# DIAGNijmegen/bodyct-dram-emph-subtype

Measured on AMD Instinct MI355X. Metric: CT volumes/sec (train step, 1x128x256x256), higher is better.
Workload: dtype f32; 1 GPU; BASELINE configs[1]: resnet18segcls train step (fwd+loss+bwd+Adam), batch 2/GPU, 1x128x256x256, fp32, inputs resident in HBM; global_batch=2, parallelism=dp1, hip_graph=False, streams=2

## Files before the change

### bodyct-dram-emph-subtype_amd/csrc/bn.hip

```cpp
#include <stdlib.h>
#include <atomic>
#include "common.h"

namespace {

template <typename T>
__global__ void reduce_partials_kernel(const T* __restrict__ partial, double* __restrict__ out, int nparts,
                                       int RC, double tail, int has_tail) {
  __shared__ double sm[256];
  const int col = blockIdx.x * 64 + (threadIdx.x & 63);
  const int lane4 = threadIdx.x >> 6;
  const int S = gridDim.y, sidx = blockIdx.y;
  double s = 0.0;
  if (col < RC)
    for (int p = sidx + S * lane4; p < nparts; p += 4 * S) s += (double)partial[(long)p * RC + col];
  sm[threadIdx.x] = s;
  __syncthreads();
  if (lane4 == 0 && col < RC)
    out[(long)sidx * RC + col] = sm[threadIdx.x] + sm[threadIdx.x + 64] + sm[threadIdx.x + 128] + sm[threadIdx.x + 192];
  if (has_tail && blockIdx.x == 0 && blockIdx.y == 0 && threadIdx.x == 0) out[RC] = tail;
}

__global__ void bn_finalize_kernel(const double* __restrict__ sums, double count_host,
                                   const double* __restrict__ count_dev, const float* __restrict__ gamma,
                                   const float* __restrict__ beta, float* __restrict__ rmean,
                                   float* __restrict__ rvar, float momentum, float eps, int update,
                                   float* __restrict__ mean, float* __restrict__ invstd, float* __restrict__ scale,
                                   float* __restrict__ shift, int C) {
  const int c = blockIdx.x * blockDim.x + threadIdx.x;
  if (c >= C) return;
  double m, v;
  const double count = count_dev ? *count_dev : count_host;
  if (sums) {
    m = sums[c] / count;
    v = sums[C + c] / count - m * m;
    if (v < 0.0) v = 0.0;
    if (update) {
      const double unb = count > 1.0 ? v * (count / (count - 1.0)) : v;
      rmean[c] = (float)((1.0 - (double)momentum) * (double)rmean[c] + (double)momentum * m);
      rvar[c] = (float)((1.0 - (double)momentum) * (double)rvar[c] + (double)momentum * unb);
    }
  } else {
    m = (double)rmean[c];
    v = (double)rvar[c];
  }
  const double is = 1.0 / sqrt(v + (double)eps);
  const float sc = (float)((double)gamma[c] * is);
  mean[c] = (float)m;
  invstd[c] = (float)is;
  scale[c] = sc;
  shift[c] = (float)((double)beta[c] - m * (double)gamma[c] * is);
}

struct FoldFinalize {
  double count;
  const float* gamma; const float* beta; float* rmean; float* rvar;
  float momentum, eps; int update;
  float* mean; float* invstd; float* scale; float* shift;
};
constexpr int FOLD_XMAX = 512;

__global__ __launch_bounds__(1024) void fold_partials_kernel(const float* __restrict__ partial, double* scratch,
                                                             double* __restrict__ sums, float* __restrict__ sums_f32,
                                                             float* __restrict__ f32_row1, const int nparts, const int RC,
                                                             const double tail,
                                                             const int has_tail, unsigned* __restrict__ ticket,
                                                             const FoldFinalize ff) {
  __shared__ double sm[1024];
  __shared__ double tot[64];
  __shared__ unsigned s_ticket;
  const int t64 = threadIdx.x & 63, lane4 = threadIdx.x >> 6;
  const int C = RC >> 1;
  const int col = ff.gamma ? (t64 >> 5) * C + blockIdx.x * 32 + (t64 & 31) : blockIdx.x * 64 + t64;
  const bool live = ff.gamma ? (blockIdx.x * 32 + (t64 & 31) < C) : (col < RC);
  const int S = gridDim.y, sidx = blockIdx.y;
  double s = 0.0;
  if (live) {
    const int step = 16 * S;
    int p = sidx + S * lane4;
    for (; p + 7 * step < nparts; p += 8 * step) {
      float v[8];
#pragma unroll
      for (int j = 0; j < 8; ++j) v[j] = partial[(long)(p + j * step) * RC + col];
#pragma unroll
      for (int j = 0; j < 8; ++j) s += (double)v[j];
    }
    for (; p < nparts; p += step) s += (double)partial[(long)p * RC + col];
  }
  sm[threadIdx.x] = s;
  __syncthreads();
  double total = 0.0;
  if (lane4 == 0) {
#pragma unroll
    for (int j = 0; j < 16; ++j) total += sm[t64 + 64 * j];
  }
  if (S > 1) {
    if (lane4 == 0 && live) scratch[(long)sidx * RC + col] = total;
    __threadfence();
    __syncthreads();
    if (threadIdx.x == 0) s_ticket = atomicAdd(&ticket[blockIdx.x], 1u);
    __syncthreads();
    if (s_ticket != (unsigned)S - 1) return;
    __threadfence();
    if (lane4 == 0 && live) {
      total = 0.0;
      int k = 0;
      for (; k + 8 <= S; k += 8) {
        double v[8];
#pragma unroll
        for (int j = 0; j < 8; ++j)
          v[j] = __hip_atomic_load(scratch + (long)(k + j) * RC + col, __ATOMIC_RELAXED, __HIP_MEMORY_SCOPE_AGENT);
#pragma unroll
        for (int j = 0; j < 8; ++j) total += v[j];
      }
      for (; k < S; ++k)
        total += __hip_atomic_load(scratch + (long)k * RC + col, __ATOMIC_RELAXED, __HIP_MEMORY_SCOPE_AGENT);
    }
  }
  if (lane4 == 0 && live) {
    sums[col] = total;
    if (sums_f32) {
      if (f32_row1 && col >= C) f32_row1[col - C] = (float)total;
      else sums_f32[col] = (float)total;
    }
  }
  if (has_tail && blockIdx.x == 0 && threadIdx.x == 0) sums[RC] = tail;
  if (!ff.gamma) return;
  if (lane4 == 0) tot[t64] = total;
  __syncthreads();
  const int c = blockIdx.x * 32 + threadIdx.x;
  if (threadIdx.x < 32 && c < C) {
    const double m = tot[threadIdx.x] / ff.count;
    double v = tot[32 + threadIdx.x] / ff.count - m * m;
    if (v < 0.0) v = 0.0;
    if (ff.update) {
      const double unb = ff.count > 1.0 ? v * (ff.count / (ff.count - 1.0)) : v;
      ff.rmean[c] = (float)((1.0 - (double)ff.momentum) * (double)ff.rmean[c] + (double)ff.momentum * m);
      ff.rvar[c] = (float)((1.0 - (double)ff.momentum) * (double)ff.rvar[c] + (double)ff.momentum * unb);
    }
    const double is = 1.0 / sqrt(v + (double)ff.eps);
    ff.mean[c] = (float)m;
    ff.invstd[c] = (float)is;
    ff.scale[c] = (float)((double)ff.gamma[c] * is);
    ff.shift[c] = (float)((double)ff.beta[c] - m * (double)ff.gamma[c] * is);
  }
}

template <int RES, typename T>
__global__ void bn_apply_kernel(const T* __restrict__ y, const float* __restrict__ scale,
                                const float* __restrict__ shift, const T* __restrict__ res, int Cr, int rs,
                                T* __restrict__ z, int D, int H, int W, int C, long total4, int relu) {
  const int Q = C >> 2;
  for (long i = blockIdx.x * (long)blockDim.x + threadIdx.x; i < total4; i += (long)gridDim.x * blockDim.x) {
    const int q = (int)(i % Q);
    const float4 sc = *reinterpret_cast<const float4*>(scale + 4 * q);
    const float4 sh = *reinterpret_cast<const float4*>(shift + 4 * q);
    const float4 v = ld4<T>(y, 4 * i);
    float4 o;
    o.x = __builtin_fmaf(v.x, sc.x, sh.x); o.y = __builtin_fmaf(v.y, sc.y, sh.y);
    o.z = __builtin_fmaf(v.z, sc.z, sh.z); o.w = __builtin_fmaf(v.w, sc.w, sh.w);
    if (RES == 1) {
      const float4 rr = ld4<T>(res, 4 * i);
      o.x += rr.x; o.y += rr.y; o.z += rr.z; o.w += rr.w;
    }
    if (relu) { o.x = fmaxf(o.x, 0.f); o.y = fmaxf(o.y, 0.f); o.z = fmaxf(o.z, 0.f); o.w = fmaxf(o.w, 0.f); }
    st4<T>(z, 4 * i, o);
  }
}

template <int RES, typename T, int U>
__global__ __launch_bounds__(256) void bn_apply_fast_kernel(const T* __restrict__ y, const float* __restrict__ scale,
                                                            const float* __restrict__ shift, const T* __restrict__ res,
                                                            T* __restrict__ z, int Q, long total4, int relu) {
  const int q = threadIdx.x % Q;
  const float4 sc = *reinterpret_cast<const float4*>(scale + 4 * q);
  const float4 sh = *reinterpret_cast<const float4*>(shift + 4 * q);
  const long stride = (long)gridDim.x * 256;
  for (long i0 = blockIdx.x * 256L + threadIdx.x; i0 < total4; i0 += U * stride) {
    float4 v[U], rr[U];
#pragma unroll
    for (int u = 0; u < U; ++u) {
      const long i = i0 + u * stride;
      if (i < total4) {
        v[u] = ld4<T>(y, 4 * i);
        if (RES == 1) rr[u] = ld4<T>(res, 4 * i);
// ... 333 lines not shown
            gg.z = zv.z > 0.f ? gg.z : 0.f; gg.w = zv.w > 0.f ? gg.w : 0.f;
          }
          const float4 o = make_float4(sc.x * gg.x, sc.y * gg.y, sc.z * gg.z, sc.w * gg.w);
          st4<T>(dy, 4 * i, o);
          cs.x += o.x; cs.y += o.y; cs.z += o.z; cs.w += o.w;
        }
      }
    }
  }
  if (colpart) {
    __shared__ float4 sm[256];
    sm[threadIdx.x] = cs;
    __syncthreads();
    if ((int)threadIdx.x < Q) {
      float4 t = sm[threadIdx.x];
      for (int k = threadIdx.x + Q; k < 256; k += Q) {
        const float4 u = sm[k];
        t.x += u.x; t.y += u.y; t.z += u.z; t.w += u.w;
      }
      *reinterpret_cast<float4*>(colpart + (long)blockIdx.x * C + 4 * threadIdx.x) = t;
    }
  }
}

__global__ void add_kernel(const float4* __restrict__ a, const float4* __restrict__ b, float4* __restrict__ o,
                           long n4, const float* __restrict__ as, const float* __restrict__ bs,
                           float* __restrict__ os, long n) {
  for (long i = blockIdx.x * (long)blockDim.x + threadIdx.x; i < n4; i += (long)gridDim.x * blockDim.x) {
    const float4 u = a[i], v = b[i];
    o[i] = make_float4(u.x + v.x, u.y + v.y, u.z + v.z, u.w + v.w);
  }
  const long t0 = n4 * 4;
  for (long i = t0 + blockIdx.x * (long)blockDim.x + threadIdx.x; i < n; i += (long)gridDim.x * blockDim.x)
    os[i] = as[i] + bs[i];
}

inline int ew_grid(long total4) {
  long b = (total4 + 255) / 256;
  return (int)(b > 4096 ? 4096 : (b < 1 ? 1 : b));
}

inline int rows_per_block(long long rows) {
  long long rpb = (rows + 1023) / 1024;
  if (rpb < 64) rpb = 64;
  return (int)rpb;
}

}

extern "C" int dram_reduce_partials_stages(int nparts) {
  if (nparts <= 64) return 1;
  int s = (nparts + 31) / 32;
  return s > 64 ? 64 : s;
}

extern "C" int dram_reduce_partials(const float* partial, double* sums, double* scratch, int nparts, int R, int C,
                                    double tail, int has_tail, dram_stream_t stream) {
  if (!partial || !sums || nparts < 1 || R < 1 || C < 1) return DRAM_ERR_BAD_ARG;
  const int RC = R * C;
  const int S = dram_reduce_partials_stages(nparts);
  hipStream_t st = (hipStream_t)stream;
  DramProf prof(DRAM_FAM_BN, 0, 0.0, 4.0 * (double)nparts * RC + 8.0 * RC, st);
  if (S == 1) {
    hipLaunchKernelGGL((reduce_partials_kernel<float>), dim3((RC + 63) / 64, 1), dim3(256), 0, st, partial, sums,
                       nparts, RC, tail, has_tail);
  } else {
    if (!scratch) return DRAM_ERR_WORKSPACE;
    hipLaunchKernelGGL((reduce_partials_kernel<float>), dim3((RC + 63) / 64, S), dim3(256), 0, st, partial, scratch,
                       nparts, RC, 0.0, 0);
    DRAM_LAUNCH_CHECK();
    hipLaunchKernelGGL((reduce_partials_kernel<double>), dim3((RC + 63) / 64, 1), dim3(256), 0, st,
                       (const double*)scratch, sums, S, RC, tail, has_tail);
  }
  DRAM_LAUNCH_CHECK();
  return DRAM_OK;
}

extern "C" int dram_fold_partials_stages(int nparts) {
  if (nparts <= 1024) return 1;
  const int s = (nparts + 511) / 512;
  return s > 64 ? 64 : s;
}

static int fold_launch(const float* partial, double* sums, double* scratch, float* sums_f32, float* f32_row1, int nparts,
                       int RC, double tail, int has_tail, const FoldFinalize& ff, hipStream_t st) {
  const int S = dram_fold_partials_stages(nparts);
  const int gx = ff.gamma ? (RC / 2 + 31) / 32 : (RC + 63) / 64;
  if (S > 1 && gx > FOLD_XMAX) return DRAM_ERR_UNSUPPORTED;
  unsigned* ticket = nullptr;
  if (S > 1) {
    ticket = reinterpret_cast<unsigned*>(scratch + (long)S * RC);
    const hipError_t e = hipMemsetAsync(ticket, 0, sizeof(unsigned) * gx, st);
    if (e != hipSuccess) return (int)e;
  }
  DramProf prof(DRAM_FAM_BN, 0, 0.0, 4.0 * (double)nparts * RC + 8.0 * RC, st);
  hipLaunchKernelGGL(fold_partials_kernel, dim3(gx, S), dim3(1024), 0, st, partial, scratch, sums, sums_f32, f32_row1,
                     nparts, RC, tail, has_tail, ticket, ff);
  DRAM_LAUNCH_CHECK();
  return DRAM_OK;
}

extern "C" int dram_fold_partials(const float* partial, double* sums, double* scratch, float* sums_f32, float* f32_row1,
                                  int nparts, int R, int C, double tail, int has_tail, dram_stream_t stream) {
  if (!partial || !sums || !scratch || nparts < 1 || R < 1 || C < 1) return DRAM_ERR_BAD_ARG;
  if (f32_row1 && (R != 2 || !sums_f32)) return DRAM_ERR_BAD_ARG;
  FoldFinalize ff{};
  return fold_launch(partial, sums, scratch, sums_f32, f32_row1, nparts, R * C, tail, has_tail, ff, (hipStream_t)stream);
}

extern "C" int dram_bn_fold_finalize(const float* partial, double* sums, double* scratch, int nparts, int C, double count,
                                     const float* gamma, const float* beta, float* running_mean, float* running_var,
                                     float momentum, float eps, int update_running, float* mean, float* invstd,
                                     float* scale, float* shift, dram_stream_t stream) {
  if (!partial || !sums || !scratch || nparts < 1 || C < 1 || count <= 0.0) return DRAM_ERR_BAD_ARG;
  if (!gamma || !beta || !mean || !invstd || !scale || !shift) return DRAM_ERR_BAD_ARG;
  if (update_running && (!running_mean || !running_var)) return DRAM_ERR_BAD_ARG;
  FoldFinalize ff{count, gamma, beta, running_mean, running_var, momentum, eps, update_running, mean, invstd, scale, shift};
  return fold_launch(partial, sums, scratch, nullptr, nullptr, nparts, 2 * C, 0.0, 0, ff, (hipStream_t)stream);
}

extern "C" int dram_bn_finalize(const double* sums, double count, const double* count_dev, const float* gamma,
                                const float* beta,
                                float* running_mean, float* running_var, float momentum, float eps,
                                int update_running, float* mean, float* invstd, float* scale, float* shift, int C,
                                dram_stream_t stream) {
  if (!gamma || !beta || !mean || !invstd || !scale || !shift || C < 1) return DRAM_ERR_BAD_ARG;
  if (!sums && (!running_mean || !running_var)) return DRAM_ERR_BAD_ARG;
  if (sums && !count_dev && count <= 0.0) return DRAM_ERR_BAD_ARG;
  if (update_running && (!running_mean || !running_var)) return DRAM_ERR_BAD_ARG;
  DramProf prof(DRAM_FAM_BN, 1, 0.0, 4.0 * 10.0 * C, (hipStream_t)stream);
  hipLaunchKernelGGL(bn_finalize_kernel, dim3((C + 255) / 256), dim3(256), 0, (hipStream_t)stream, sums, count,
                     count_dev, gamma, beta, running_mean, running_var, momentum, eps, update_running, mean, invstd, scale,
                     shift, C);
  DRAM_LAUNCH_CHECK();
  return DRAM_OK;
}

template <typename T>
static int bn_apply_impl(const T* y, const float* scale, const float* shift, const T* residual, int Dr, int Hr, int Wr,
                         int Cr, int rs, T* z, int B, int D, int H, int W, int C, int relu, dram_stream_t stream) {
  if (!y || !scale || !shift || !z || B < 1 || D < 1 || H < 1 || W < 1 || C < 4 || (C & 3)) return DRAM_ERR_BAD_ARG;
  const long total4 = (long)B * D * H * W * (C >> 2);
  hipStream_t s = (hipStream_t)stream;
  const int grid = ew_blocks(total4, 256, 4096);
  const double res_frac = !residual ? 0.0 : ((double)Cr / C) / ((double)rs * rs * rs);
  DramProf prof(DRAM_FAM_BN, 2, 0.0, 4.0 * sizeof(T) * (double)total4 * (2.0 + res_frac), s);
  const int Q = C >> 2;
  const bool identity = residual && rs == 1 && Cr == C && Dr == D && Hr == H && Wr == W;
  static const int ew_u = tune_env("DRAM_EW_U") ? atoi(tune_env("DRAM_EW_U")) : 4;
  if ((!residual || identity) && 256 % Q == 0 && ew_u > 0 && ew_shape() > 0) {
    const int g1 = ew_blocks(total4, 1024, 0);
#define BN_SHOT_(RES_, NT_) hipLaunchKernelGGL((bn_apply_shot_kernel<RES_, T, NT_>), dim3(g1), dim3(256), 0, s, y, scale, \
                                               shift, residual, z, Q, total4, relu)
    const bool nt = ew_stream(sizeof(T) * 4 * total4);
    if (!residual) { if (nt) BN_SHOT_(0, true); else BN_SHOT_(0, false); }
    else           { if (nt) BN_SHOT_(1, true); else BN_SHOT_(1, false); }
#undef BN_SHOT_
  } else if ((!residual || identity) && 256 % Q == 0 && ew_u > 0) {
    const long per = (total4 + 255) / 256;
    const int g2 = (int)((per + ew_u - 1) / ew_u < 8192 ? ((per + ew_u - 1) / ew_u < 1 ? 1 : (per + ew_u - 1) / ew_u) : 8192);
#define BN_FAST_(RES_, U_) hipLaunchKernelGGL((bn_apply_fast_kernel<RES_, T, U_>), dim3(g2), dim3(256), 0, s, y, scale, shift, \
                                              residual, z, Q, total4, relu)
    if (!residual) { if (ew_u >= 4) BN_FAST_(0, 4); else if (ew_u >= 2) BN_FAST_(0, 2); else BN_FAST_(0, 1); }
    else           { if (ew_u >= 4) BN_FAST_(1, 4); else if (ew_u >= 2) BN_FAST_(1, 2); else BN_FAST_(1, 1); }
#undef BN_FAST_
  } else if (!residual) {
    hipLaunchKernelGGL((bn_apply_kernel<0, T>), dim3(grid), dim3(256), 0, s, y, scale, shift, (const T*)nullptr, 0,
                       1, z, D, H, W, C, total4, relu);
  } else if (identity) {
    hipLaunchKernelGGL((bn_apply_kernel<1, T>), dim3(grid), dim3(256), 0, s, y, scale, shift, residual,
                       Cr, 1, z, D, H, W, C, total4, relu);
  } else {
    if ((Cr & 3) || Cr < 4 || Cr > C || rs < 1) return DRAM_ERR_BAD_ARG;
    if ((D - 1) * rs >= Dr || (H - 1) * rs >= Hr || (W - 1) * rs >= Wr) return DRAM_ERR_BAD_ARG;
    hipLaunchKernelGGL((bn_apply_shortcut_a_kernel<T>), dim3(grid), dim3(256), 0, s, y, scale, shift,
                       residual, Dr, Hr, Wr, Cr, rs, z, D, H, W, C, total4, relu);
// ... 159 lines not shown
```

### bodyct-dram-emph-subtype_amd/csrc/common.h

```cpp
#pragma once
#include <hip/hip_runtime.h>
#include <stdint.h>
#include <stdlib.h>
#include "dram_hip.h"

typedef float f32x16 __attribute__((ext_vector_type(16)));
typedef float f32x4 __attribute__((ext_vector_type(4)));

#define DRAM_LAUNCH_CHECK()                         \
  do {                                              \
    hipError_t _e = hipGetLastError();              \
    if (_e != hipSuccess) return (int)_e;           \
  } while (0)

extern bool g_dram_prof_on;
void dram_prof_begin(int family, int variant, double mfma_flops, double hbm_bytes, double alg_flops, hipStream_t s);
void dram_prof_end(hipStream_t s);
struct DramProf {
  const bool on;
  hipStream_t s;
  DramProf(int family, int variant, double mfma_flops, double hbm_bytes, hipStream_t st, double alg_flops = -1.0)
      : on(g_dram_prof_on), s(st) {
    if (on) dram_prof_begin(family, variant, mfma_flops, hbm_bytes, alg_flops < 0.0 ? mfma_flops : alg_flops, st);
  }
// ... 43 lines not shown
template <> __device__ __forceinline__ fvec<4> ldv<float, 4>(const float* p, long off) {
  const float4 t = *reinterpret_cast<const float4*>(p + off);
  return fvec<4>{{t.x, t.y, t.z, t.w}};
}
template <> __device__ __forceinline__ fvec<4> ldv<bf16_t, 4>(const bf16_t* p, long off) {
  const uint2 u = *reinterpret_cast<const uint2*>(p + off);
  return fvec<4>{{__uint_as_float(u.x << 16), __uint_as_float(u.x & 0xffff0000u), __uint_as_float(u.y << 16),
                  __uint_as_float(u.y & 0xffff0000u)}};
}
template <> __device__ __forceinline__ fvec<8> ldv<bf16_t, 8>(const bf16_t* p, long off) {
  const uint4 u = *reinterpret_cast<const uint4*>(p + off);
  return fvec<8>{{__uint_as_float(u.x << 16), __uint_as_float(u.x & 0xffff0000u), __uint_as_float(u.y << 16),
                  __uint_as_float(u.y & 0xffff0000u), __uint_as_float(u.z << 16), __uint_as_float(u.z & 0xffff0000u),
                  __uint_as_float(u.w << 16), __uint_as_float(u.w & 0xffff0000u)}};
}
template <typename T, int VW> __device__ __forceinline__ void stv(T* p, long off, const fvec<VW>& a);
template <> __device__ __forceinline__ void stv<float, 4>(float* p, long off, const fvec<4>& a) {
  *reinterpret_cast<float4*>(p + off) = make_float4(a.v[0], a.v[1], a.v[2], a.v[3]);
}
template <> __device__ __forceinline__ void stv<bf16_t, 4>(bf16_t* p, long off, const fvec<4>& a) {
  *reinterpret_cast<uint2*>(p + off) = make_uint2(pack2_bf16(a.v[0], a.v[1]), pack2_bf16(a.v[2], a.v[3]));
}
template <> __device__ __forceinline__ void stv<bf16_t, 8>(bf16_t* p, long off, const fvec<8>& a) {
  *reinterpret_cast<uint4*>(p + off) = make_uint4(pack2_bf16(a.v[0], a.v[1]), pack2_bf16(a.v[2], a.v[3]),
                                                  pack2_bf16(a.v[4], a.v[5]), pack2_bf16(a.v[6], a.v[7]));
}

typedef float f32x4_nt __attribute__((ext_vector_type(4)));
typedef unsigned u32x2_nt __attribute__((ext_vector_type(2)));
template <typename T> __device__ __forceinline__ float4 ld4s(const T* p, long off);
template <> __device__ __forceinline__ float4 ld4s<float>(const float* p, long off) {
  const f32x4_nt t = __builtin_nontemporal_load(reinterpret_cast<const f32x4_nt*>(p + off));
  return make_float4(t.x, t.y, t.z, t.w);
}
template <> __device__ __forceinline__ float4 ld4s<bf16_t>(const bf16_t* p, long off) {
  const u32x2_nt u = __builtin_nontemporal_load(reinterpret_cast<const u32x2_nt*>(p + off));
  return make_float4(__uint_as_float(u.x << 16), __uint_as_float(u.x & 0xffff0000u), __uint_as_float(u.y << 16),
                     __uint_as_float(u.y & 0xffff0000u));
}
template <typename T> __device__ __forceinline__ void st4s(T* p, long off, float4 v);
template <> __device__ __forceinline__ void st4s<float>(float* p, long off, float4 v) {
  const f32x4_nt t = {v.x, v.y, v.z, v.w};
  __builtin_nontemporal_store(t, reinterpret_cast<f32x4_nt*>(p + off));
}
template <> __device__ __forceinline__ void st4s<bf16_t>(bf16_t* p, long off, float4 v) {
  const u32x2_nt t = {pack2_bf16(v.x, v.y), pack2_bf16(v.z, v.w)};
  __builtin_nontemporal_store(t, reinterpret_cast<u32x2_nt*>(p + off));
}

static inline const char* tune_env(const char* name) {
  static const bool on = [] { const char* t = getenv("DRAM_TUNING"); return t && t[0] == '1'; }();
  return on ? getenv(name) : nullptr;
}

static inline int ew_shape() {
  static const int v = tune_env("DRAM_EW_SHAPE") ? atoi(tune_env("DRAM_EW_SHAPE")) : 2;
  return v;
}
static inline bool ew_stream(long long tensor_bytes) { return ew_shape() >= 2 && tensor_bytes >= (256LL << 20); }
static inline int ew_blocks(long items, int per_block, int cap) {
  long b = (items + per_block - 1) / per_block;
  if (b < 1) b = 1;
  if (ew_shape() == 0 && b > cap) b = cap;
  return (int)(b > 0x7fffffffL ? 0x7fffffffL : b);
}

static inline int cdiv(long long a, long long b) { return (int)((a + b - 1) / b); }

__device__ __forceinline__ int xcd_remap(int bid, int nblk) {
  const int q = nblk >> 3, r = nblk & 7;
  const int xcd = bid & 7, idx = bid >> 3;
  return (xcd < r ? xcd * (q + 1) : r * (q + 1) + (xcd - r) * q) + idx;
}

__device__ __forceinline__ void lin_src(int dst, float scale, int in, int& i0, int& i1, float& w0, float& w1) {
  const float s = scale * (float)dst;
  i0 = (int)s;
  if (i0 > in - 1) i0 = in - 1;
  i1 = i0 + (i0 < in - 1 ? 1 : 0);
  w1 = s - (float)i0;
  w0 = 1.f - w1;
}

__device__ __forceinline__ float wave_sum(float v) {
#pragma unroll
  for (int o = 32; o > 0; o >>= 1) v += __shfl_xor(v, o, 64);
  return v;
}
```

### bodyct-dram-emph-subtype_amd/csrc/pool_up.hip

```cpp
#include <stdlib.h>
#include <string.h>
#include <initializer_list>
#include "common.h"

namespace {

inline int ew_grid(long total) { return ew_blocks(total, 256, 8192); }

template <typename T, int VW>
__global__ void maxpool_fwd_kernel(const T* __restrict__ x, T* __restrict__ y,
                                   uint8_t* __restrict__ amax, int D, int H, int W, int C, int Do, int Ho, int Wo,
                                   long total) {
  const int Q = C / VW;
  for (long i = blockIdx.x * (long)blockDim.x + threadIdx.x; i < total; i += (long)gridDim.x * blockDim.x) {
    const int q = (int)(i % Q);
    long v = i / Q;
    const int xo = (int)(v % Wo); v /= Wo;
    const int yo = (int)(v % Ho); v /= Ho;
    const int zo = (int)(v % Do);
    const long b = v / Do;
    fvec<VW> m;
    int am[VW];
#pragma unroll
    for (int k = 0; k < VW; ++k) { m.v[k] = -INFINITY; am[k] = 0; }
// ... 266 lines not shown
template <typename T, int VW>
__global__ __launch_bounds__(256) void upcat_fwd_tiled_kernel(const T* __restrict__ src, const T* __restrict__ skip,
                                                              T* __restrict__ cat, int Ds, int Hs, int Ws, int Cu,
                                                              int Dk, int Hk, int Wk, int Ck, int oz, int oy, int ox,
                                                              float sz, float sy, float sx, int tz_n, int ty_n,
                                                              int tx_n) {
  constexpr int LPV = 64 / VW;
  constexpr int SLOTS = 256 / LPV;
  __shared__ float4 tile[216 * 16];
  const int Do = 2 * Ds, Ho = 2 * Hs, Wo = 2 * Ws;
  const int Ct = Cu + Ck, Qk = Ck / VW;
  int r = blockIdx.x;
  const int txi = r % tx_n; r /= tx_n;
  const int tyi = r % ty_n; r /= ty_n;
  const int tzi = r % tz_n;
  const long b = r / tz_n;
  const int z0 = tzi * 8, y0 = tyi * 8, x0 = txi * 8;
  int zb, yb, xb, d1;
  float w0, w1;
  lin_src(z0, sz, Ds, zb, d1, w0, w1);
  lin_src(y0, sy, Hs, yb, d1, w0, w1);
  lin_src(x0, sx, Ws, xb, d1, w0, w1);
  const int tid = threadIdx.x, q = tid % LPV, vs = tid / LPV;
  for (int cb = 0; cb < Cu; cb += 64) {
    __syncthreads();
    for (int e = tid; e < 216 * LPV; e += 256) {
      const int qq = e % LPV, v = e / LPV;
      const int lx = v % 6, ly = (v / 6) % 6, lz = v / 36;
      const int zz = min(zb + lz, Ds - 1), yy = min(yb + ly, Hs - 1), xx = min(xb + lx, Ws - 1);
      const fvec<VW> t = ldv<T, VW>(src, (((b * Ds + zz) * Hs + yy) * Ws + xx) * (long)Cu + cb + VW * qq);
#pragma unroll
      for (int k = 0; k < VW; k += 4)
        tile[v * 16 + (VW / 4) * qq + (k >> 2)] = make_float4(t.v[k], t.v[k + 1], t.v[k + 2], t.v[k + 3]);
    }
    __syncthreads();
    for (int v = vs; v < 512; v += SLOTS) {
      const int zo = z0 + (v >> 6), yo = y0 + ((v >> 3) & 7), xo = x0 + (v & 7);
      if (zo >= Do || yo >= Ho || xo >= Wo) continue;
      int za, zc, ya, yc, xa, xc;
      float wz0, wz1, wy0, wy1, wx0, wx1;
      lin_src(zo, sz, Ds, za, zc, wz0, wz1);
      lin_src(yo, sy, Hs, ya, yc, wy0, wy1);
      lin_src(xo, sx, Ws, xa, xc, wx0, wx1);
      za -= zb; zc -= zb; ya -= yb; yc -= yb; xa -= xb; xc -= xb;
      fvec<VW> o;
#pragma unroll
      for (int k = 0; k < VW; ++k) o.v[k] = 0.f;
#define UPT_ACC(zz, yy, xx, ww)                                                              \
  {                                                                                          \
    const float w_ = (ww);                                                                   \
    _Pragma("unroll") for (int k = 0; k < VW; k += 4) {                                      \
      const float4 t = tile[(((zz) * 6 + (yy)) * 6 + (xx)) * 16 + (VW / 4) * q + (k >> 2)];  \
      o.v[k] += w_ * t.x; o.v[k + 1] += w_ * t.y; o.v[k + 2] += w_ * t.z; o.v[k + 3] += w_ * t.w; \
    }                                                                                        \
  }
      UPT_ACC(za, ya, xa, wz0 * wy0 * wx0) UPT_ACC(za, ya, xc, wz0 * wy0 * wx1)
      UPT_ACC(za, yc, xa, wz0 * wy1 * wx0) UPT_ACC(za, yc, xc, wz0 * wy1 * wx1)
      UPT_ACC(zc, ya, xa, wz1 * wy0 * wx0) UPT_ACC(zc, ya, xc, wz1 * wy0 * wx1)
      UPT_ACC(zc, yc, xa, wz1 * wy1 * wx0) UPT_ACC(zc, yc, xc, wz1 * wy1 * wx1)
#undef UPT_ACC
      const long vox = ((b * Do + zo) * Ho + yo) * (long)Wo + xo;
      stv<T, VW>(cat, vox * Ct + cb + VW * q, o);
    }
  }
  for (int e = tid; e < 512 * Qk; e += 256) {
    const int qq = e % Qk, v = e / Qk;
    const int zo = z0 + (v >> 6), yo = y0 + ((v >> 3) & 7), xo = x0 + (v & 7);
    if (zo >= Do || yo >= Ho || xo >= Wo) continue;
    const long vox = ((b * Do + zo) * Ho + yo) * (long)Wo + xo;
    stv<T, VW>(cat, vox * Ct + Cu + VW * qq,
               ldv<T, VW>(skip, (((b * Dk + zo + oz) * Hk + yo + oy) * Wk + xo + ox) * (long)Ck + VW * qq));
  }
}

__device__ __forceinline__ void dst_range(int s, float scale, int out, int& lo, int& hi) {
  if (scale <= 0.f) { lo = 0; hi = out - 1; return; }
  const float inv = 1.f / scale;
  lo = (int)floorf((float)(s - 1) * inv) - 1;
  hi = (int)ceilf((float)(s + 1) * inv) + 1;
  if (lo < 0) lo = 0;
  if (hi > out - 1) hi = out - 1;
}

struct UpAxis {
  int lo;
  float w[6];
};
__device__ __forceinline__ UpAxis up_axis(int s, float scale, int in, int out) {
  UpAxis t;
  int lo = scale > 0.f ? (int)floorf((float)(s - 1) / scale) - 1 : 0;
  if (lo < 0) lo = 0;
  t.lo = lo;
#pragma unroll
  for (int j = 0; j < 6; ++j) {
    const int d = lo + j;
    int a0, a1;
    float u0, u1;
    lin_src(d, scale, in, a0, a1, u0, u1);
    const float w = (a0 == s ? u0 : 0.f) + (a1 == s ? u1 : 0.f);
    t.w[j] = d < out ? w : 0.f;
  }
  return t;
}

template <typename T, int VW>
__global__ void upcat_bwd_src_kernel(const T* __restrict__ dcat, T* __restrict__ dsrc, int Ds, int Hs, int Ws,
                                     int Cu, int Ct, float sz, float sy, float sx, long total) {
  const int Do = 2 * Ds, Ho = 2 * Hs, Wo = 2 * Ws;
  const int Qu = Cu / VW;
  for (long i = blockIdx.x * (long)blockDim.x + threadIdx.x; i < total; i += (long)gridDim.x * blockDim.x) {
    const int q = (int)(i % Qu);
    long v = i / Qu;
    const int xs = (int)(v % Ws); v /= Ws;
    const int ys = (int)(v % Hs); v /= Hs;
    const int zs = (int)(v % Ds);
    const long b = v / Ds;
    const UpAxis tz = up_axis(zs, sz, Ds, Do), ty = up_axis(ys, sy, Hs, Ho), tx = up_axis(xs, sx, Ws, Wo);
    fvec<VW> acc;
#pragma unroll
    for (int k = 0; k < VW; ++k) acc.v[k] = 0.f;
#pragma unroll
    for (int jz = 0; jz < 6; ++jz) {
      if (tz.w[jz] == 0.f) continue;
#pragma unroll
      for (int jy = 0; jy < 6; ++jy) {
        const float wzy = tz.w[jz] * ty.w[jy];
        if (wzy == 0.f) continue;
        const T* row = dcat + (((b * Do + tz.lo + jz) * Ho + ty.lo + jy) * (long)Wo + tx.lo) * (long)Ct + VW * q;
        fvec<VW> g[6];
#pragma unroll
        for (int jx = 0; jx < 6; ++jx)
          g[jx] = ldv<T, VW>(row, (long)(tx.w[jx] != 0.f ? jx : 0) * Ct);
#pragma unroll
        for (int jx = 0; jx < 6; ++jx) {
          const float w_ = wzy * tx.w[jx];
#pragma unroll
          for (int k = 0; k < VW; ++k) acc.v[k] = __builtin_fmaf(w_, g[jx].v[k], acc.v[k]);
        }
      }
    }
    stv<T, VW>(dsrc, VW * i, acc);
  }
}

template <typename T, int VW>
__global__ void upcat_bwd_skip_kernel(const T* __restrict__ dcat, T* __restrict__ dskip, int Do, int Ho,
                                      int Wo, int Cu, int Dk, int Hk, int Wk, int Ck, int oz, int oy, int ox,
                                      long total) {
  const int Qk = Ck / VW;
  const int Ct = Cu + Ck;
  for (long i = blockIdx.x * (long)blockDim.x + threadIdx.x; i < total; i += (long)gridDim.x * blockDim.x) {
    const int q = (int)(i % Qk);
    long v = i / Qk;
    const int xk = (int)(v % Wk); v /= Wk;
    const int yk = (int)(v % Hk); v /= Hk;
    const int zk = (int)(v % Dk);
    const long b = v / Dk;
    const int zo = zk - oz, yo = yk - oy, xo = xk - ox;
    fvec<VW> o;
#pragma unroll
    for (int k = 0; k < VW; ++k) o.v[k] = 0.f;
    if (zo >= 0 && zo < Do && yo >= 0 && yo < Ho && xo >= 0 && xo < Wo)
      o = ldv<T, VW>(dcat, (((b * Do + zo) * Ho + yo) * Wo + xo) * (long)Ct + Cu + VW * q);
    stv<T, VW>(dskip, VW * i, o);
  }
}

__global__ __launch_bounds__(256) void upproject_kernel(const float* __restrict__ dense, const float* __restrict__ ess,
                                                        float* __restrict__ out, float* __restrict__ partial, int D,
                                                        int H, int W, int Do, int Ho, int Wo, float sz, float sy,
                                                        float sx, long vps, int nblk) {
  __shared__ float sm[4];
  const int b = blockIdx.y;
  float s = 0.f;
  for (long v = blockIdx.x * (long)blockDim.x + threadIdx.x; v < vps; v += (long)gridDim.x * blockDim.x) {
    long r = v;
    const int xo = (int)(r % Wo); r /= Wo;
    const int yo = (int)(r % Ho);
    const int zo = (int)(r / Ho);
    int z0, z1, y0, y1, x0, x1;
    float wz0, wz1, wy0, wy1, wx0, wx1;
    lin_src(zo, sz, D, z0, z1, wz0, wz1);
    lin_src(yo, sy, H, y0, y1, wy0, wy1);
    lin_src(xo, sx, W, x0, x1, wx0, wx1);
    const float* p = dense + (long)b * D * H * W;
#define DV(zz, yy, xx) p[((long)(zz) * H + (yy)) * W + (xx)]
// ... 79 lines not shown
}

template <typename T>
static int maxpool_bwd_impl(const T* dy, const uint8_t* argmax, const T* add, int add_stride, T* dx, int B, int D, int H,
                            int W, int C, dram_stream_t stream) {
  if (!dy || !dx || !argmax || B < 1 || D < 1 || H < 1 || W < 1 || C < 4 || (C & 3)) return DRAM_ERR_BAD_ARG;
  if (add && (add_stride < C || (add_stride & 3) || ((uintptr_t)add & (4 * sizeof(T) - 1)))) return DRAM_ERR_BAD_ARG;
  const int Do = (D + 2 - 3) / 2 + 1, Ho = (H + 2 - 3) / 2 + 1, Wo = (W + 2 - 3) / 2 + 1;
  const long total4 = (long)B * D * H * W * (C >> 2);
  DramProf prof(DRAM_FAM_POOL_UP, 1, 0.0,
                (double)sizeof(T) * 4.0 * total4 * (1.0 + (add ? 1 : 0)) + (1.0 + sizeof(T)) * (double)B * Do * Ho * Wo * C,
                (hipStream_t)stream);
  const bool wide = pool_wide(sizeof(T), {C, add ? add_stride : 0, (add && ((uintptr_t)add & 15)) ? 1 : 0});
  static const bool per_voxel = tune_env("DRAM_POOL_BWD") && !strcmp(tune_env("DRAM_POOL_BWD"), "voxel");
  if (!per_voxel) {
    const long totb = (long)B * ((D + 1) / 2) * ((H + 1) / 2) * ((W + 1) / 2) * (C / (wide ? 8 : 4));
    POOL_LAUNCH(wide, maxpool_bwd_blk_kernel, ew_grid(totb), dy, argmax, add, add_stride, dx, D, H, W, C, Do, Ho, Wo, totb);
    DRAM_LAUNCH_CHECK();
    return DRAM_OK;
  }
  const long total = wide ? total4 / 2 : total4;
  POOL_LAUNCH(wide, maxpool_bwd_kernel, ew_grid(total), dy, argmax, add, add_stride, dx, D, H, W, C, Do, Ho, Wo, total);
  DRAM_LAUNCH_CHECK();
  return DRAM_OK;
}
extern "C" int dram_maxpool_bwd(const float* dy, const uint8_t* argmax, const float* add, int add_stride, float* dx,
                                int B, int D, int H, int W, int C, dram_stream_t stream) {
  return maxpool_bwd_impl<float>(dy, argmax, add, add_stride, dx, B, D, H, W, C, stream);
}
extern "C" int dram_maxpool_bwd_bf16(const void* dy, const uint8_t* argmax, const void* add, int add_stride, void* dx,
                                     int B, int D, int H, int W, int C, dram_stream_t stream) {
  return maxpool_bwd_impl<bf16_t>((const bf16_t*)dy, argmax, (const bf16_t*)add, add_stride, (bf16_t*)dx, B, D, H, W, C,
                                  stream);
}

template <typename T>
static int upcat_fwd_impl(const T* src, const T* skip, T* cat, int B, int Ds, int Hs, int Ws, int Cu, int Dk, int Hk,
                          int Wk, int Ck, dram_stream_t stream) {
  if (!src || !cat || B < 1 || Cu < 4 || (Cu & 3) || (skip ? (Ck < 4 || (Ck & 3)) : Ck != 0)) return DRAM_ERR_BAD_ARG;
  const int Do = 2 * Ds, Ho = 2 * Hs, Wo = 2 * Ws;
  if (Dk < Do || Hk < Ho || Wk < Wo) return DRAM_ERR_BAD_ARG;
  const int oz = (Dk - Do + 1) / 2, oy = (Hk - Ho + 1) / 2, ox = (Wk - Wo + 1) / 2;
  const long total4 = (long)B * Do * Ho * Wo * ((Cu + Ck) >> 2);
  const long tiles = (long)B * ((Do + 7) / 8) * ((Ho + 7) / 8) * ((Wo + 7) / 8);
  DramProf prof(DRAM_FAM_POOL_UP, 2, 0.0,
                (double)sizeof(T) * ((double)B * Ds * Hs * Ws * Cu + (double)B * Do * Ho * Wo * Ck + 4.0 * total4),
                (hipStream_t)stream);
  const bool wide = pool_wide(sizeof(T), {Cu, Ck});
  if (Cu % 64 == 0 && tiles >= 512 && tiles < (1L << 31) && !tune_env("DRAM_UPCAT_UNTILED")) {
    POOL_LAUNCH(wide, upcat_fwd_tiled_kernel, (unsigned)tiles, src, skip, cat, Ds, Hs, Ws, Cu, Dk, Hk, Wk, Ck, oz, oy, ox,
                ac_scale(Ds, Do), ac_scale(Hs, Ho), ac_scale(Ws, Wo), (Do + 7) / 8, (Ho + 7) / 8, (Wo + 7) / 8);
    DRAM_LAUNCH_CHECK();
    return DRAM_OK;
  }
  const long total = wide ? total4 / 2 : total4;
  POOL_LAUNCH(wide, upcat_fwd_kernel, ew_grid(total), src, skip, cat, Ds, Hs, Ws, Cu, Dk, Hk, Wk, Ck, oz, oy, ox,
              ac_scale(Ds, Do), ac_scale(Hs, Ho), ac_scale(Ws, Wo), total);
  DRAM_LAUNCH_CHECK();
  return DRAM_OK;
}
extern "C" int dram_upcat_fwd(const float* src, const float* skip, float* cat, int B, int Ds, int Hs, int Ws, int Cu,
                              int Dk, int Hk, int Wk, int Ck, dram_stream_t stream) {
  return upcat_fwd_impl<float>(src, skip, cat, B, Ds, Hs, Ws, Cu, Dk, Hk, Wk, Ck, stream);
}
extern "C" int dram_upcat_fwd_bf16(const void* src, const void* skip, void* cat, int B, int Ds, int Hs, int Ws, int Cu,
                                   int Dk, int Hk, int Wk, int Ck, dram_stream_t stream) {
  return upcat_fwd_impl<bf16_t>((const bf16_t*)src, (const bf16_t*)skip, (bf16_t*)cat, B, Ds, Hs, Ws, Cu, Dk, Hk, Wk, Ck,
                                stream);
}

template <typename T>
static int upcat_bwd_impl(const T* dcat, T* dsrc, T* dskip, int B, int Ds, int Hs, int Ws, int Cu, int Dk, int Hk, int Wk,
                          int Ck, dram_stream_t stream) {
  if (!dcat || (!dsrc && !dskip) || B < 1 || Cu < 4 || Ck < 4 || (Cu & 3) || (Ck & 3)) return DRAM_ERR_BAD_ARG;
  const int Do = 2 * Ds, Ho = 2 * Hs, Wo = 2 * Ws;
  if (Dk < Do || Hk < Ho || Wk < Wo) return DRAM_ERR_BAD_ARG;
  const int oz = (Dk - Do + 1) / 2, oy = (Hk - Ho + 1) / 2, ox = (Wk - Wo + 1) / 2;
  hipStream_t s = (hipStream_t)stream;
  const bool wide = pool_wide(sizeof(T), {Cu, Ck});
  if (dsrc) {
    const long total4 = (long)B * Ds * Hs * Ws * (Cu >> 2);
    DramProf prof(DRAM_FAM_POOL_UP, 3, 0.0, (double)sizeof(T) * ((double)B * Do * Ho * Wo * Cu + 4.0 * total4), s);
    const long total = wide ? total4 / 2 : total4;
    POOL_LAUNCH(wide, upcat_bwd_src_kernel, ew_grid(total), dcat, dsrc, Ds, Hs, Ws, Cu, Cu + Ck, ac_scale(Ds, Do),
                ac_scale(Hs, Ho), ac_scale(Ws, Wo), total);
    DRAM_LAUNCH_CHECK();
  }
  if (dskip) {
    const long total4 = (long)B * Dk * Hk * Wk * (Ck >> 2);
    DramProf prof(DRAM_FAM_POOL_UP, 4, 0.0, (double)sizeof(T) * ((double)B * Do * Ho * Wo * Ck + 4.0 * total4), s);
    const long total = wide ? total4 / 2 : total4;
    POOL_LAUNCH(wide, upcat_bwd_skip_kernel, ew_grid(total), dcat, dskip, Do, Ho, Wo, Cu, Dk, Hk, Wk, Ck, oz, oy, ox,
                total);
    DRAM_LAUNCH_CHECK();
  }
  return DRAM_OK;
}
extern "C" int dram_upcat_bwd(const float* dcat, float* dsrc, float* dskip, int B, int Ds, int Hs, int Ws, int Cu,
                              int Dk, int Hk, int Wk, int Ck, dram_stream_t stream) {
  return upcat_bwd_impl<float>(dcat, dsrc, dskip, B, Ds, Hs, Ws, Cu, Dk, Hk, Wk, Ck, stream);
}
extern "C" int dram_upcat_bwd_bf16(const void* dcat, void* dsrc, void* dskip, int B, int Ds, int Hs, int Ws, int Cu,
                                   int Dk, int Hk, int Wk, int Ck, dram_stream_t stream) {
  return upcat_bwd_impl<bf16_t>((const bf16_t*)dcat, (bf16_t*)dsrc, (bf16_t*)dskip, B, Ds, Hs, Ws, Cu, Dk, Hk, Wk, Ck,
                                stream);
}

extern "C" int dram_upproject_nblk(long long vps) {
  long long b = (vps + 1023) / 1024;
  return (int)(b > 1024 ? 1024 : (b < 1 ? 1 : b));
}

extern "C" int dram_upproject(const float* dense, const float* ess, float* out, float* partial, int B, int D, int H,
                              int W, int Do, int Ho, int Wo, dram_stream_t stream) {
  if (!dense || !ess || !out || !partial || B < 1 || D < 1 || H < 1 || W < 1 || Do < 1 || Ho < 1 || Wo < 1)
    return DRAM_ERR_BAD_ARG;
  const long vps = (long)Do * Ho * Wo;
  const int nblk = dram_upproject_nblk(vps);
  DramProf prof(DRAM_FAM_POOL_UP, 5, 0.0, 4.0 * ((double)B * D * H * W + 2.0 * B * (double)vps), (hipStream_t)stream);
  hipLaunchKernelGGL(upproject_kernel, dim3(nblk, B), dim3(256), 0, (hipStream_t)stream, dense, ess, out, partial, D, H,
                     W, Do, Ho, Wo, ac_scale(D, Do), ac_scale(H, Ho), ac_scale(W, Wo), vps, nblk);
  DRAM_LAUNCH_CHECK();
  return DRAM_OK;
}
```

Measured before the change: 54.78 volumes/sec.

## Tile upcat backward through shared-memory planes and persist fold tickets

Adds a tiled upcat-backward kernel. Each block stages a 13x13x64-channel plane of the upsampled gradient in LDS for successive depth slices, then accumulates 4x4x4 source voxels from it, so dcat is no longer re-read from global memory for every overlapping source voxel. Separately, the BN fold kernel now draws its ticket counters from a persistent per-stream device arena and resets them inside the kernel. This removes a hipMemsetAsync before each multi-stage fold launch. The costs are added complexity, the register-staged prefetch, and host-side map lookups, plus stream capture queries on each launch.

Measured after the change: 55.08 volumes/sec, median of 6. About the same (+0.5%).

```diff
diff --git a/bodyct-dram-emph-subtype_amd/csrc/bn.hip b/bodyct-dram-emph-subtype_amd/csrc/bn.hip
--- a/bodyct-dram-emph-subtype_amd/csrc/bn.hip
+++ b/bodyct-dram-emph-subtype_amd/csrc/bn.hip
@@ -1,5 +1,10 @@
 #include <stdlib.h>
+#include <string.h>
 #include <atomic>
+#include <map>
+#include <mutex>
+#include <tuple>
+#include <utility>
 #include "common.h"
 
 namespace {
@@ -59,6 +64,8 @@
   float* mean; float* invstd; float* scale; float* shift;
 };
 constexpr int FOLD_XMAX = 512;
+constexpr int FOLD_SLOTS = 64;
+__device__ unsigned g_fold_tickets[FOLD_SLOTS * FOLD_XMAX];
 
 __global__ __launch_bounds__(1024) void fold_partials_kernel(const float* __restrict__ partial, double* scratch,
                                                              double* __restrict__ sums, float* __restrict__ sums_f32,
@@ -101,6 +108,7 @@
     if (threadIdx.x == 0) s_ticket = atomicAdd(&ticket[blockIdx.x], 1u);
     __syncthreads();
     if (s_ticket != (unsigned)S - 1) return;
+    if (threadIdx.x == 0) ticket[blockIdx.x] = 0u;
     __threadfence();
     if (lane4 == 0 && live) {
       total = 0.0;
@@ -600,6 +608,39 @@
   return s > 64 ? 64 : s;
 }
 
+static unsigned* fold_tickets(hipStream_t st) {
+  if (const char* e = tune_env("DRAM_FOLD_TICKETS")) { if (!strcmp(e, "memset")) return nullptr; }
+  struct Key {
+    int dev; hipStream_t st; unsigned long long cap;
+    bool operator<(const Key& o) const { return std::tie(dev, st, cap) < std::tie(o.dev, o.st, o.cap); }
+  };
+  static std::mutex mu;
+  static std::map<Key, unsigned*> slots;
+  static std::map<int, std::pair<unsigned*, int>> arenas;
+  Key k{0, st, 0ULL};
+  if (hipGetDevice(&k.dev) != hipSuccess) return nullptr;
+  hipStreamCaptureStatus cs = hipStreamCaptureStatusNone;
+  unsigned long long id = 0;
+  if (hipStreamGetCaptureInfo(st, &cs, &id) != hipSuccess) { (void)hipGetLastError(); return nullptr; }
+  if (cs == hipStreamCaptureStatusActive) k.cap = id + 1;
+  std::lock_guard<std::mutex> lock(mu);
+  auto it = slots.find(k);
+  if (it != slots.end()) return it->second;
+  auto ar = arenas.find(k.dev);
+  if (ar == arenas.end()) {
+    void* base = nullptr;
+    if (hipGetSymbolAddress(&base, HIP_SYMBOL(g_fold_tickets)) != hipSuccess || !base) {
+      (void)hipGetLastError();
+      return nullptr;
+    }
+    ar = arenas.emplace(k.dev, std::make_pair(static_cast<unsigned*>(base), 0)).first;
+  }
+  if (ar->second.second >= FOLD_SLOTS) return nullptr;
+  unsigned* p = ar->second.first + (long)FOLD_XMAX * ar->second.second++;
+  slots.emplace(k, p);
+  return p;
+}
+
 static int fold_launch(const float* partial, double* sums, double* scratch, float* sums_f32, float* f32_row1, int nparts,
                        int RC, double tail, int has_tail, const FoldFinalize& ff, hipStream_t st) {
   const int S = dram_fold_partials_stages(nparts);
@@ -607,9 +648,12 @@
   if (S > 1 && gx > FOLD_XMAX) return DRAM_ERR_UNSUPPORTED;
   unsigned* ticket = nullptr;
   if (S > 1) {
-    ticket = reinterpret_cast<unsigned*>(scratch + (long)S * RC);
-    const hipError_t e = hipMemsetAsync(ticket, 0, sizeof(unsigned) * gx, st);
-    if (e != hipSuccess) return (int)e;
+    ticket = fold_tickets(st);
+    if (!ticket) {
+      ticket = reinterpret_cast<unsigned*>(scratch + (long)S * RC);
+      const hipError_t e = hipMemsetAsync(ticket, 0, sizeof(unsigned) * gx, st);
+      if (e != hipSuccess) return (int)e;
+    }
   }
   DramProf prof(DRAM_FAM_BN, 0, 0.0, 4.0 * (double)nparts * RC + 8.0 * RC, st);
   hipLaunchKernelGGL(fold_partials_kernel, dim3(gx, S), dim3(1024), 0, st, partial, scratch, sums, sums_f32, f32_row1,
diff --git a/bodyct-dram-emph-subtype_amd/csrc/common.h b/bodyct-dram-emph-subtype_amd/csrc/common.h
--- a/bodyct-dram-emph-subtype_amd/csrc/common.h
+++ b/bodyct-dram-emph-subtype_amd/csrc/common.h
@@ -149,6 +149,30 @@
   w0 = 1.f - w1;
 }
 
+struct UpAxis {
+  int lo;
+  float w[6];
+};
+__device__ __forceinline__ UpAxis up_axis(int s, float scale, int in, int out) {
+  UpAxis t;
+  int lo = scale > 0.f ? (int)floorf((float)(s - 1) / scale) - 1 : 0;
+  if (lo < 0) lo = 0;
+  t.lo = lo;
+#pragma unroll
+  for (int j = 0; j < 6; ++j) {
+    const int d = lo + j;
+    int a0, a1;
+    float u0, u1;
+    lin_src(d, scale, in, a0, a1, u0, u1);
+    const float w = (a0 == s ? u0 : 0.f) + (a1 == s ? u1 : 0.f);
+    t.w[j] = d < out ? w : 0.f;
+  }
+  return t;
+}
+
+int upcat_bwd_src_tiled_launch(const float* dcat, float* dsrc, int B, int Ds, int Hs, int Ws, int Cu, int Ct, float sz,
+                               float sy, float sx, hipStream_t stream);
+
 __device__ __forceinline__ float wave_sum(float v) {
 #pragma unroll
   for (int o = 32; o > 0; o >>= 1) v += __shfl_xor(v, o, 64);
diff --git a/bodyct-dram-emph-subtype_amd/csrc/pool_up.hip b/bodyct-dram-emph-subtype_amd/csrc/pool_up.hip
--- a/bodyct-dram-emph-subtype_amd/csrc/pool_up.hip
+++ b/bodyct-dram-emph-subtype_amd/csrc/pool_up.hip
@@ -372,26 +372,6 @@
   if (hi > out - 1) hi = out - 1;
 }
 
-struct UpAxis {
-  int lo;
-  float w[6];
-};
-__device__ __forceinline__ UpAxis up_axis(int s, float scale, int in, int out) {
-  UpAxis t;
-  int lo = scale > 0.f ? (int)floorf((float)(s - 1) / scale) - 1 : 0;
-  if (lo < 0) lo = 0;
-  t.lo = lo;
-#pragma unroll
-  for (int j = 0; j < 6; ++j) {
-    const int d = lo + j;
-    int a0, a1;
-    float u0, u1;
-    lin_src(d, scale, in, a0, a1, u0, u1);
-    const float w = (a0 == s ? u0 : 0.f) + (a1 == s ? u1 : 0.f);
-    t.w[j] = d < out ? w : 0.f;
-  }
-  return t;
-}
 
 template <typename T, int VW>
 __global__ void upcat_bwd_src_kernel(const T* __restrict__ dcat, T* __restrict__ dsrc, int Ds, int Hs, int Ws,
@@ -637,9 +617,24 @@
     const long total4 = (long)B * Ds * Hs * Ws * (Cu >> 2);
     DramProf prof(DRAM_FAM_POOL_UP, 3, 0.0, (double)sizeof(T) * ((double)B * Do * Ho * Wo * Cu + 4.0 * total4), s);
     const long total = wide ? total4 / 2 : total4;
-    POOL_LAUNCH(wide, upcat_bwd_src_kernel, ew_grid(total), dcat, dsrc, Ds, Hs, Ws, Cu, Cu + Ck, ac_scale(Ds, Do),
-                ac_scale(Hs, Ho), ac_scale(Ws, Wo), total);
-    DRAM_LAUNCH_CHECK();
+    bool launched = false;
+    const int tzn = (Ds + 3) / 4, tyn = (Hs + 3) / 4, txn = (Ws + 3) / 4;
+    const long tiles = (long)B * tzn * tyn * txn;
+    bool tiled = tiles * (Cu / 64) >= 256;
+    if (const char* e = tune_env("DRAM_UPCAT_BWD")) tiled = !strcmp(e, "tiled") || (tiled && strcmp(e, "untiled"));
+    if constexpr (sizeof(T) == 4) {
+      if (tiled && Cu % 64 == 0 && Cu / 64 <= 65535 && tiles < (1L << 31) && (long)Ho * Wo * (Cu + Ck) < (1L << 31)) {
+        const int rc = upcat_bwd_src_tiled_launch(dcat, dsrc, B, Ds, Hs, Ws, Cu, Cu + Ck, ac_scale(Ds, Do),
+                                                  ac_scale(Hs, Ho), ac_scale(Ws, Wo), s);
+        if (rc != DRAM_OK) return rc;
+        launched = true;
+      }
+    }
+    if (!launched) {
+      POOL_LAUNCH(wide, upcat_bwd_src_kernel, ew_grid(total), dcat, dsrc, Ds, Hs, Ws, Cu, Cu + Ck, ac_scale(Ds, Do),
+                  ac_scale(Hs, Ho), ac_scale(Ws, Wo), total);
+      DRAM_LAUNCH_CHECK();
+    }
   }
   if (dskip) {
     const long total4 = (long)B * Dk * Hk * Wk * (Ck >> 2);
diff --git a/bodyct-dram-emph-subtype_amd/csrc/upcat_bwd_tiled.hip b/bodyct-dram-emph-subtype_amd/csrc/upcat_bwd_tiled.hip
--- /dev/null
+++ b/bodyct-dram-emph-subtype_amd/csrc/upcat_bwd_tiled.hip
@@ -0,0 +1,111 @@
+#include <math.h>
+#include "common.h"
+
+namespace {
+
+__device__ __forceinline__ int up_axis_lo(int s, float scale) {
+  const int lo = scale > 0.f ? (int)floorf((float)(s - 1) / scale) - 1 : 0;
+  return lo < 0 ? 0 : lo;
+}
+
+constexpr int UPB_E = 13;
+__global__ __launch_bounds__(256)
+void upcat_bwd_src_tiled_kernel(const float* __restrict__ dcat, float* __restrict__ dsrc, int Ds, int Hs, int Ws, int Cu,
+                                int Ct, float sz, float sy, float sx, int tz_n, int ty_n, int tx_n) {
+  constexpr int E = UPB_E, NE = E * E * 16, NL = (NE + 255) / 256;
+  __shared__ float4 plane[NE];
+  const int Do = 2 * Ds, Ho = 2 * Hs, Wo = 2 * Ws;
+  int r = blockIdx.x;
+  const int txi = r % tx_n; r /= tx_n;
+  const int tyi = r % ty_n; r /= ty_n;
+  const int tzi = r % tz_n;
+  const long b = r / tz_n;
+  const int cb = blockIdx.y * 64;
+  const int tid = threadIdx.x, q = tid & 15, lx = (tid >> 4) & 3, ly = tid >> 6;
+  const int zs0 = tzi * 4, ys = tyi * 4 + ly, xs = txi * 4 + lx;
+  const bool live = ys < Hs && xs < Ws;
+  const UpAxis ty = up_axis(min(ys, Hs - 1), sy, Hs, Ho), tx = up_axis(min(xs, Ws - 1), sx, Ws, Wo);
+  const int oy0 = up_axis_lo(tyi * 4, sy), ox0 = up_axis_lo(txi * 4, sx);
+  const int py = min(ty.lo - oy0, E - 6), px = min(tx.lo - ox0, E - 6);
+  int lok[4];
+#pragma unroll
+  for (int k = 0; k < 4; ++k) lok[k] = up_axis_lo(min(zs0 + k, Ds - 1), sz);
+  const int dlo = lok[0], dhi = min(lok[3] + 5, Do - 1);
+
+  fvec<4> acc[4];
+#pragma unroll
+  for (int k = 0; k < 4; ++k)
+#pragma unroll
+    for (int c = 0; c < 4; ++c) acc[k].v[c] = 0.f;
+
+  float4 stage[NL];
+  auto fetch = [&](int d) {
+    const float* base = dcat + ((b * Do + d) * Ho) * (long)Wo * Ct + cb;
+#pragma unroll
+    for (int i = 0; i < NL; ++i) {
+      const int e = tid + 256 * i, v = e >> 4;
+      const int gy = oy0 + v / E, gx = ox0 + v % E;
+      const bool ok = e < NE && gy < Ho && gx < Wo;
+      const int off = ok ? (gy * Wo + gx) * Ct + 4 * (e & 15) : -1;
+      stage[i] = off >= 0 ? *reinterpret_cast<const float4*>(base + off) : make_float4(0.f, 0.f, 0.f, 0.f);
+    }
+  };
+  fetch(dlo);
+  for (int d = dlo; d <= dhi; ++d) {
+    __syncthreads();
+#pragma unroll
+    for (int i = 0; i < NL; ++i) {
+      const int e = tid + 256 * i;
+      if (e < NE) plane[e] = stage[i];
+    }
+    __syncthreads();
+    if (d < dhi) fetch(d + 1);
+    int a0, a1;
+    float u0, u1;
+    lin_src(d, sz, Ds, a0, a1, u0, u1);
+#pragma unroll
+    for (int k = 0; k < 4; ++k) {
+      const int s = zs0 + k, jz = d - lok[k];
+      float wz = (a0 == s ? u0 : 0.f) + (a1 == s ? u1 : 0.f);
+      if (s >= Ds || jz < 0 || jz >= 6) wz = 0.f;
+      if (wz == 0.f || !live) continue;
+#pragma unroll
+      for (int jy = 0; jy < 6; ++jy) {
+        const float wzy = wz * ty.w[jy];
+        if (wzy == 0.f) continue;
+        const float4* row = plane + ((py + jy) * E + px) * 16 + q;
+        float4 g[6];
+#pragma unroll
+        for (int jx = 0; jx < 6; ++jx) g[jx] = row[(tx.w[jx] != 0.f ? jx : 0) * 16];
+#pragma unroll
+        for (int jx = 0; jx < 6; ++jx) {
+          const float w_ = wzy * tx.w[jx];
+          acc[k].v[0] = __builtin_fmaf(w_, g[jx].x, acc[k].v[0]);
+          acc[k].v[1] = __builtin_fmaf(w_, g[jx].y, acc[k].v[1]);
+          acc[k].v[2] = __builtin_fmaf(w_, g[jx].z, acc[k].v[2]);
+          acc[k].v[3] = __builtin_fmaf(w_, g[jx].w, acc[k].v[3]);
+        }
+      }
+    }
+  }
+  if (!live) return;
+#pragma unroll
+  for (int k = 0; k < 4; ++k)
+    if (zs0 + k < Ds)
+      stv<float, 4>(dsrc, ((((b * Ds + zs0 + k) * Hs + ys) * Ws + xs) * (long)Cu) + cb + 4 * q, acc[k]);
+}
+
+}
+
+int upcat_bwd_src_tiled_launch(const float* dcat, float* dsrc, int B, int Ds, int Hs, int Ws, int Cu, int Ct, float sz,
+                               float sy, float sx, hipStream_t stream) {
+  if (!dcat || !dsrc || B < 1 || Ds < 1 || Hs < 1 || Ws < 1 || Cu < 64 || Cu % 64 || Ct < Cu || (Ct & 3))
+    return DRAM_ERR_BAD_ARG;
+  const int tzn = (Ds + 3) / 4, tyn = (Hs + 3) / 4, txn = (Ws + 3) / 4;
+  const long tiles = (long)B * tzn * tyn * txn;
+  if (tiles >= (1L << 31) || Cu / 64 > 65535 || 4L * Hs * Ws * Ct >= (1L << 31)) return DRAM_ERR_UNSUPPORTED;
+  hipLaunchKernelGGL(upcat_bwd_src_tiled_kernel, dim3((unsigned)tiles, Cu / 64), dim3(256), 0, stream, dcat, dsrc, Ds, Hs,
+                     Ws, Cu, Ct, sz, sy, sx, tzn, tyn, txn);
+  DRAM_LAUNCH_CHECK();
+  return DRAM_OK;
+}
```
